# antarcticrainforest/seabreeze_param

Hardware: AMD Instinct MI355X
Metric: grid-points/sec for sea_breeze_diag on N2560x1920 global grid; achieved HBM GB/s (higher is better)
Workload: dtype f64; 1 GPU; seabreeze_diag generic flavour, N1280 (2560x1920) global grid, nz=56, fp64 (BASELINE.json configs[2]); stream=torch's current stream (torch and the library share one HIP runtime), plan_cache=stored, nx=2560, ny=1920, nz=56, search_halo=16, parallelism=latband1, variant=default, comm=none, multi_rank_rccl=unmeasured on hardware so far (one GPU per box in the build pool)

## Files before the change

seabreeze_param_amd/csrc/sb_capi.hip:

```cpp
#include "../../include/seabreeze_hip.h"
#include "sb_launch.hpp"

#include <dlfcn.h>
#include <rccl/rccl.h>

#include <algorithm>
#include <chrono>
#include <cmath>
#include <condition_variable>
#include <functional>
#include <mutex>
#include <thread>
#include <cstdio>
#include <cstdlib>
#include <cstring>
#include <string>
#include <vector>

namespace {

thread_local std::string g_err;

struct DevBuf {
    void *p = nullptr;
// ... 198 lines not shown
           c->stats_ngathered == (c->gathered ? c->ngathered : 0);
}

template <typename T>
int run_diag(sb_ctx *c, DiagJob<T> &job, hipStream_t st, int phases = 3) {
    const Geo &g = job.g;
    const size_t ncell = (size_t)g.nxh * g.nyh;
    const size_t nbits = (size_t)g.nyh * g.nw * sizeof(uint64_t);
    int rc;
    if ((rc = ensure(c, c->bandbits, nbits))) return rc;
    if ((rc = ensure(c, c->clsbits, nbits))) return rc;
    const int H = pick_halo(c);
    int txw, tyrows, tx, ty;
    const bool strip32 = H > 16 && sizeof(T) == 4 && !c->no_wide_strip && sb_strip32_shape(g.nx, g.rows, &tx, &ty);
    const bool strip = strip32 || (H <= 16 && sb_strip_shape(g.nx, g.rows, &tx, &ty));
    const int vb = strip32 ? 2 : 1;
    if (strip) { txw = 32; tyrows = 16; }
    else {
        sb_thc_tile_shape(H > 16 ? H : 24, &txw, &tyrows);
        tx = (g.nx + txw - 1) / txw; ty = (g.rows + tyrows - 1) / tyrows;
    }
    const int Hk = strip32 ? 32 : strip ? 16 : (H > 16 ? H : 24);
    const int ntile = strip ? tx * (ty + 2 * vb) : tx * ty;
    const int nflag = ntile + 2;
    if (c->tiles.cap < (size_t)2 * nflag * sizeof(int) || c->tiles_n != nflag || c->tiles_strip != (strip ? vb : 0)) {
        if ((rc = ensure(c, c->tiles, (size_t)2 * nflag * sizeof(int)))) return rc;
        HIPCHK(c, hipMemsetAsync(c->tiles.p, 0, (size_t)2 * nflag * sizeof(int), st));
        c->tiles_n = nflag;
        c->tiles_strip = strip ? vb : 0;
        c->flag_parity = 0;
    }
    int *flags_now = (int *)c->tiles.p + (size_t)c->flag_parity * nflag;
    int *flags_next = (int *)c->tiles.p + (size_t)(1 - c->flag_parity) * nflag;
    job.thc_ty = tyrows; job.thc_ntx = tx; job.thc_nty = ty;
    job.thc_txs = txw == 32 ? 5 : 6;
    job.strip = strip32 ? 2 : strip ? 1 : 0;
    if (strip) { job.tile_sx = ty + 2 * vb; job.tile_sy = 1; job.tile_off = vb; }
    else { job.tile_sx = 1; job.tile_sy = tx; job.tile_off = 0; }
    job.bandbits = (uint64_t *)c->bandbits.p;
    job.clsbits = (uint64_t *)c->clsbits.p;
    job.stats = (const T *)c->stats;
    job.tile_nnmax = flags_now;
    job.counters = flags_now + (size_t)ntile;
    job.ticket = (int *)c->ticket;
// ... 16 lines not shown
        if ((rc = ensure(c, c->nws, (size_t)g.nx * g.ny * sizeof(T)))) return rc;
        if ((rc = ensure(c, c->nwd, (size_t)g.nx * g.ny * sizeof(T)))) return rc;
        job.nws = (T *)c->nws.p;
        job.nwd = (T *)c->nwd.p;
    }
    job.t0 = nullptr;
    if (!job.t0_fly) {
        if ((rc = ensure(c, c->t0, ncell * sizeof(T)))) return rc;
        job.t0 = (T *)c->t0.p;
    }
    if ((rc = ensure(c, c->jobcopy, sizeof(DiagJob<double>)))) return rc;
    job.self = (DiagJob<T> *)c->jobcopy.p;
    job.plan = nullptr; job.plan_gen = nullptr; job.call_id = 0; job.plan_use = 0; job.seg_trust = 0;
    job.moments_out = nullptr; job.stats_ticket = nullptr; job.strip_update = 0;
    if (strip) {
        const size_t need = 64 + (size_t)c->ncu * SB_PLAN_STRIDE;
        if (c->plan.cap < need) {
            if ((rc = ensure(c, c->plan, need))) return rc;
            HIPCHK(c, hipMemsetAsync(c->plan.p, 0, need, st));
            c->plan_bits = nullptr;
        }
        if (phases & 1) {
            if (c->call_seq == 0x7fffffff) {
                HIPCHK(c, hipMemsetAsync(c->plan.p, 0, need, st));
                c->call_seq = 0;
                c->plan_bits = nullptr;
            }
            ++c->call_seq;
            const int key[8] = {g.nx, g.ny, g.h, g.bnd, g.rows, c->ncu, tx, ty | (vb << 24)};
            c->plan_use = c->plan_bits == c->bandbits.p && std::memcmp(key, c->plan_key, sizeof(key)) == 0 ? 1 : 0;
            std::memcpy(c->plan_key, key, sizeof(key));
            c->plan_bits = c->bandbits.p;
        }
        job.plan = (char *)c->plan.p + 64;
        job.plan_gen = (int *)c->plan.p;
        job.call_id = c->call_seq;
        job.plan_use = c->no_plan_cache ? 0 : c->plan_use;
    } else if (phases & 1) c->plan_bits = nullptr;
    job.stamps = nullptr;
#ifdef SB_STAMPS
    if ((rc = ensure(c, c->stamps, (size_t)4096 * SB_NSTAMP * sizeof(long long)))) return rc;
    job.stamps = (long long *)c->stamps.p;
#endif
    SbLaunchCtx lc;
// ... 1356 lines not shown
```

seabreeze_param_amd/csrc/sb_launch.hpp:

```cpp
#pragma once
#include "sb_device.hpp"

#define SB_STATS_MAX_BLOCKS 2048
#define SB_MAX_LDS_HALO 32
#define SB_DIST_TY 4
enum { SB_PROF_SCAN = 0, SB_PROF_WIND = 1, SB_PROF_T0 = 2, SB_PROF_THC = 3, SB_PROF_PREP = 4, SB_PROF_KERNELS = 5 };
#define SB_PROF_EVENTS (2 * SB_PROF_KERNELS)
#ifndef SB_WIND_UN
#define SB_WIND_UN 8
#endif
#ifndef SB_WIND_WGS_PER_CU
#define SB_WIND_WGS_PER_CU 4
#endif
#ifndef SB_WIND_UN_F32
#define SB_WIND_UN_F32 14
#endif
#ifndef SB_WIND_WGS_PER_CU_F32
#define SB_WIND_WGS_PER_CU_F32 8
#endif

struct SbLaunchCtx {
    hipStream_t stream;
    hipEvent_t *prof;
    unsigned *prof_mask;
// ... 14 lines not shown

template <typename T>
hipError_t sb_launch_stats(const T *ary, int nx, int ny, int ld, size_t off0, Moments *partials, T *stats,
                           Moments *moments_out, int *ticket, hipStream_t st);
template <typename T>
hipError_t sb_launch_sigmoid_apply(const T *ary, T *sm, size_t n, const T *stats, hipStream_t st);
template <typename T>
hipError_t sb_launch_diag(const DiagJob<T> &job, int H, const SbLaunchCtx &lc);
void sb_thc_tile_shape(int H, int *tx, int *ty);
template <typename T>
hipError_t sb_launch_thc(const DiagJob<T> &job, int H, int ncu, hipStream_t st);

template <typename T>
hipError_t sb_launch_strip(const DiagJob<T> &job, int ncu, hipStream_t st);
bool sb_strip_shape(int nx, int rows, int *ntx, int *nty);
template <typename T>
hipError_t sb_launch_strip32(const DiagJob<T> &job, int ncu, hipStream_t st);
template <>
hipError_t sb_launch_strip32<float>(const DiagJob<float> &job, int ncu, hipStream_t st);
template <>
hipError_t sb_launch_strip32<double>(const DiagJob<double> &job, int ncu, hipStream_t st);
bool sb_strip32_shape(int nx, int rows, int *ntx, int *nty);

template <typename T>
hipError_t sb_launch_theta_to_t0(T *theta, const T *z, const T *sigma, size_t n, const T *stats, hipStream_t st);

template <typename T>
hipError_t sb_launch_edges(const T *lsm, const T *ci, T *coast, int nx, int ny, int rule, int bnd, hipStream_t st);
template <typename T>
hipError_t sb_launch_dist(const T *coast, const T *mask, const T *phi, const T *lamf,
// ... 15 lines not shown
```

seabreeze_param_amd/csrc/sb_strip_kernel.hip:

```cpp
#include "sb_thc_common.hpp"
#include "sb_strip_common.hpp"

#define STRIP_H 16
#define STRIP_W 64
#define STRIP_SW (STRIP_W - 2 * STRIP_H)
#define STRIP_C 16
#define STRIP_NT 1024
#define STRIP_RING 128
#define STRIP_P (STRIP_W + 1)
#define STRIP_MAXW 768
#define STRIP_SCHED 384
#define STRIP_ROUND 90
#define STRIP_FB 40
#define STRIP_DEPTH 3


#if defined(SB_STAMPS) && !defined(SB_STAMPS_WIND)
#define SB_T(i) do { if (lane == 0) job.stamps[(size_t)(blockIdx.x * (STRIP_NT / SB_WAVE) + wv) * SB_NSTAMP + (i)] = wall_clock64(); } while (0)
#else
#define SB_T(i) do { } while (0)
#endif

__constant__ double sb_strip_k[20] = {
    1.4426950408889634, 0.6931471805599453, 2.3190468138462996e-17, -708.0, 700.0,
    1.6666666666666666e-01, 4.1666666666666664e-02, 8.333333333333333e-03, 1.388888888888889e-03,
    1.984126984126984e-04, 2.48015873015873e-05, 2.7557319223985893e-06, 2.755731922398589e-07,
    2.505210838544172e-08,
// ... 37 lines not shown

#define SB_FIX_BIAS 0x4338000000000000ull
__device__ __forceinline__ u64 sb_to_fixed(double x, sb_cdp k) {
    return (u64)__double_as_longlong(__builtin_fma(x, SB_K(16, 0x1p40), SB_K(17, 0x1.8p52)));
}

template <typename T, bool FLY>
struct StripRegs {
    T th;
    T zz, sg;
    uint32_t lw;
    uint32_t lbit;
};

template <typename T, bool FLY>
__global__ __launch_bounds__(STRIP_NT) void k_strip(char *plan, const int *plan_gen, const Moments *fold_partials, int G, StripJob<T> job) {
    constexpr int H = STRIP_H, W = STRIP_W, SW = STRIP_SW, C = STRIP_C, P = STRIP_P, NWV = STRIP_NT / SB_WAVE;
    constexpr int RM = STRIP_RING - 1;
    static_assert(NWV == C && SW == 32, "one staged row per wave, 32 owned columns");
    static_assert(STRIP_SCHED == SB_PLAN_SCHED, "a stored plan holds one round's steps");
    __shared__ u64 sA[STRIP_RING * P];
    __shared__ u64 sL[STRIP_RING * P];
    __shared__ unsigned short sC[STRIP_RING * P];
    __shared__ u64 s_land[STRIP_RING];
    __shared__ u64 s_bits[STRIP_MAXW];
    __shared__ uint2 s_ent[STRIP_SCHED];
    __shared__ unsigned short s_cell[3][SW * C];
    __shared__ Moments s_wpart[NWV];
    __shared__ int s_scan[NWV];
    __shared__ int s_misc[12];
    __shared__ T s_sdr[2];
    static_assert(sizeof(u64) * (2 * STRIP_RING * P + STRIP_RING + STRIP_MAXW) + 2 * STRIP_RING * P + 8 * STRIP_SCHED +
                          6 * SW * C + sizeof(Moments) * NWV + 4 * NWV + 48 + 16 <= 160 * 1024,
                  "k_strip: LDS of one workgroup");

    const Geo g = job.g;
    const int tid = threadIdx.x, lane = tid & 63;
    const int wv = __builtin_amdgcn_readfirstlane(tid >> 6);
    const int npad = job.nty + 2;
    const int npos = job.ntx * npad;
    const unsigned npad_magic = 0xffffffffu / (unsigned)npad + 1u;

    SB_T(0);
    T sd = T(0), rr = T(0);
    Moments pm = moments_empty();
    double shift_c = 0.0;
    const bool fold_stats = job.fold && job.fold_nparts > 0;
    if (fold_stats) {
        if (tid < job.fold_nparts) pm = fold_partials[tid];
        shift_c = (double)job.sigma[(size_t)g.h * g.nxh + g.h];
    } else if (FLY && job.ngath > 0) {
        if (wv == 0) {
            Moments m = moments_empty();
            for (int b = lane; b < job.ngath; b += SB_WAVE) m = moments_merge(m, job.gath[b]);
// ... 4 lines not shown
                s_sdr[0] = st4[0]; s_sdr[1] = st4[1];
                if (blockIdx.x == 0) { for (int i = 0; i < 4; ++i) job.stats_out[i] = st4[i]; }
            }
        }
    } else if (FLY) { sd = job.stats[0]; rr = job.stats[1]; }
    const int nch = (npos + STRIP_NT - 1) / STRIP_NT;
    const int nwords = nch * NWV;
    typedef const __attribute__((address_space(4))) int *cintp;
    char *const plan_wg = plan + (size_t)blockIdx.x * SB_PLAN_STRIDE;
    unsigned *const plan_lists = (unsigned *)(plan_wg + SB_PLAN_LIST_OFF);
    const uint2 plan_ent = ((const uint2 *)(plan_wg + SB_PLAN_ENT_OFF))[tid < STRIP_SCHED ? tid : 0];
    const int plan_stored = ((cintp)plan_wg)[0], plan_nst = min(((cintp)plan_wg)[1], STRIP_SCHED);
    const int plan_rb = ((cintp)plan_wg)[2], plan_re = ((cintp)plan_wg)[3];
    const bool cached = job.plan_use != 0 && plan_stored != 0 && *(cintp)plan_gen <= plan_stored;
    auto load_plane = [&]() {
        u64 mine = 0;
        for (int base = 0; base < nch; base += 8) {
            int f[8];
#pragma unroll
            for (int j = 0; j < 8; ++j) {
                const int i = (base + j) * STRIP_NT + tid;
                f[j] = job.flags[i < npos ? i : npos - 1];
            }
#pragma unroll
            for (int j = 0; j < 8; ++j) {
                const int i = (base + j) * STRIP_NT + tid;
                mine |= (i < npos && f[j] != 0) ? 1ull << (base + j) : 0ull;
            }
        }
        for (int c = 0; c < nch; ++c) {
            const u64 b = __builtin_amdgcn_ballot_w64((mine >> c) & 1ull);
            if (lane == 0) s_bits[c * NWV + wv] = b;
        }
    };
    if (__builtin_expect(!cached, 0)) load_plane();
    else {
        if (tid < plan_nst) s_ent[tid] = plan_ent;
        if (tid == 0) { s_misc[0] = plan_nst; s_misc[5] = plan_rb; s_misc[6] = plan_re; s_misc[8] = 0; }
    }
    for (int i = tid; i < STRIP_RING; i += STRIP_NT) { sA[i * P] = 0; sL[i * P] = 0; sC[i * P] = 0; }
    if (tid == 0) s_misc[4] = 0;
    if (fold_stats) wave_total_shifted_store(pm, s_wpart);
    SB_T(1);
    __syncthreads();
    SB_T(2);
    unsigned *s_pre = (unsigned *)&s_cell[0][0];
    unsigned *s_cost = (unsigned *)&sA[0];
    constexpr int CW_STAGED = 4, CW_ACTIVE = 2, CW_RUN = 2;
    static_assert(sizeof(s_cell) >= sizeof(unsigned) * STRIP_MAXW, "the prefix array fits where the cell lists lie");
    auto wave_sync = [] { asm volatile("s_waitcnt lgkmcnt(0)" ::: "memory"); };
    auto stage_word = [&](int k) -> u64 {
        const u64 a = s_bits[k], pv = k > 0 ? s_bits[k - 1] : 0ull, nx = k + 1 < nwords ? s_bits[k + 1] : 0ull;
        return a | (a << 1) | (pv >> 63) | (a >> 1) | (nx << 63);
    };
    auto run_starts = [&](int k, u64 sw) -> u64 {
        const u64 swp = k > 0 ? stage_word(k - 1) : 0ull;
        return sw & ~((sw << 1) | (swp >> 63));
    };
    int tot_packed = 0, tot_cost = 0;
    auto make_prefix = [&](bool with_cost) {
        int run = 0, crun = 0;
        for (int k0 = 0; k0 < nwords; k0 += SB_WAVE) {
            const int k = k0 + lane;
            const u64 a = k < nwords ? s_bits[k] : 0ull, sw = k < nwords ? stage_word(k) : 0ull;
            const int v = (int)((unsigned)__popcll(a) | (unsigned)__popcll(sw) << 16);
            const int incl = sb_wave_scan_add(v);
            if (k < nwords) s_pre[k] = (unsigned)(run + incl - v);
            run += __builtin_amdgcn_readlane(incl, SB_WAVE - 1);
// ... 43 lines not shown
                const u64 upto = lane == 63 ? ~0ull : (1ull << (lane + 1)) - 1ull;
                const int cum = __builtin_amdgcn_readlane(lo, src) + CW_STAGED * __popcll(sw & upto) + CW_ACTIVE * __popcll(a & upto) + CW_RUN * __popcll(rs & upto);
                const u64 over = __builtin_amdgcn_ballot_w64(cum > t);
                const int bpos = over ? __ffsll((unsigned long long)over) - 1 : 63;
                return (int)(__builtin_amdgcn_readfirstlane((int)s_pre[kk]) & 0xffff) + __popcll(a & ((1ull << bpos) - 1ull));
            }
        }
        return nact;
    };
    auto make_schedule = [&](int ra, int rb) {
        int n0, n1;
        const int k0w = find_word(ra, false, n0), k1w = find_word(rb - 1, false, n1);
        const int p0 = k0w < 0 ? -1 : k0w * 64 + nth_bit(sb_uniform64(s_bits[k0w < 0 ? 0 : k0w]), n0);
        const int p1 = k1w < 0 ? -1 : k1w * 64 + nth_bit(sb_uniform64(s_bits[k1w < 0 ? 0 : k1w]), n1);
        wave_sync();
        if (p0 < 1 || p1 < p0) { if (lane == 0) s_misc[0] = 0; return; }
        if (lane < STRIP_DEPTH) s_ent[lane] = make_uint2(SCH_DRAIN | SCH_IDLE, 0u);
        if (lane < 3) s_misc[1 + lane] = 0;
        int n_out = STRIP_DEPTH;
        for (int c = p0 - 1; c <= p1 + 1; c += SB_WAVE) {
            const int pp = c + lane;
            unsigned win = 0;
#pragma unroll
            for (int d = 0; d < 5; ++d) {
                const int q = pp + d - 2;
                const bool in = q >= p0 && q <= p1;
                const u64 w = s_bits[in ? q >> 6 : 0];
                win |= (in && ((w >> (q & 63)) & 1ull)) ? 1u << d : 0u;
            }
            const bool st = pp <= p1 + 1 && (win & 0xeu) != 0u;
            const int sp = (int)__umulhi((unsigned)(pp < 0 ? 0 : pp), npad_magic), jpp = pp - sp * npad;
            const bool st_prev = (win & 0x7u) != 0u && jpp != 0, st_next = (win & 0x1cu) != 0u && jpp != npad - 1;
            const bool en = st && !st_next;
            const u64 ms = __builtin_amdgcn_ballot_w64(st), me = __builtin_amdgcn_ballot_w64(en);
            const u64 below = (1ull << lane) - 1ull;
            const int at = n_out + __popcll(ms & below) + __popcll(me & below);
            n_out += __popcll(ms) + __popcll(me);
            if (st) {
                const unsigned sjv = ((unsigned)sp << 16) | (unsigned)jpp;
                const unsigned e = (unsigned)pp | ((win & 1u) ? SCH_Q2 : 0u) | (st_prev ? 0u : SCH_RESTART);
                if (at < STRIP_SCHED) s_ent[at] = make_uint2(e, sjv);
                if (en && at + 1 < STRIP_SCHED) s_ent[at + 1] = make_uint2((unsigned)pp | SCH_DRAIN | ((win & 2u) ? SCH_Q1 : 0u), sjv);
            }
        }
        n_out = min(n_out, STRIP_SCHED - 2);
        const int n_pad = (n_out + STRIP_DEPTH - 1) / STRIP_DEPTH * STRIP_DEPTH;
        wave_sync();
        const unsigned last_sj = s_ent[n_out - 1].y;
        if (lane < n_pad - n_out) s_ent[n_out + lane] = make_uint2(SCH_DRAIN | SCH_IDLE, last_sj);
        if (lane == 0) s_misc[0] = n_pad;
    };
    if (__builtin_expect(!cached, 0)) {
        if (wv == 0) {
            make_prefix(true);
            const int rb0 = act_before_cost((int)(((long long)blockIdx.x * tot_cost) / G));
            const int re0 = blockIdx.x + 1 == (unsigned)G ? (tot_packed & 0xffff) : act_before_cost((int)(((long long)(blockIdx.x + 1) * tot_cost) / G));
            if (lane == 0) { s_misc[5] = rb0; s_misc[6] = re0; s_misc[0] = 0; }
// ... 9 lines not shown
                const u64 m = __builtin_amdgcn_ballot_w64(q);
                const int qi = nq + __popcll(m & ((1ull << lane) - 1ull));
                nq += __popcll(m);
                if (q) v.x |= (unsigned)(qi & (SB_PLAN_NQ - 1)) << SCH_QI_SHIFT;
                if (i < nstv) { s_ent[i] = v; eg[i] = v; }
            }
            const bool ok = re0 - rb0 <= STRIP_ROUND && nq <= SB_PLAN_NQ;
            if (lane == 0) {
                int *h = (int *)plan_wg;
                h[1] = nstv; h[2] = rb0; h[3] = re0;
                h[0] = ok ? job.call_id : 0;
                s_misc[8] = ok ? 1 : 0;
            }
        }
        __syncthreads();
        if (tid < 8) sA[tid * P] = 0;
        SB_T(3);
    }
    const bool store_lists = __builtin_amdgcn_readfirstlane(s_misc[8]) != 0;
    unsigned qc = ~0u;
    const unsigned qc_off = (unsigned)(min(wv, C / 2 - 1) * SB_WAVE + lane);
    const int r_begin = __builtin_amdgcn_readfirstlane(s_misc[5]), r_end = __builtin_amdgcn_readfirstlane(s_misc[6]);

    const bool fastx = g.nx > W + 2;
    const bool limited = g.bnd == BND_HALO;
    const int big_reach = 1 << 20;
    auto frame_reach = [&](int x, int y) __attribute__((always_inline)) -> int {
        const int rx = (g.band & GEO_BAND_EW) ? big_reach : min(x + g.h, g.nx - 1 - x + g.h);
        const int rs = (g.band & GEO_BAND_SOUTH) ? big_reach : y + g.h, rn = (g.band & GEO_BAND_NORTH) ? big_reach : g.ny - 1 - y + g.h;
        return min(rx, min(rs, rn));
    };
// ... 16 lines not shown
            else if (fastx) {
                if (g.bnd == BND_WRAPPER) {
                    int m = xs + 1;
                    m = m < 0 ? m + g.nx : (m >= g.nx ? m - g.nx : m);
                    Xc = (m < 1 ? 1 : m) - 1;
                } else Xc = xs < 0 ? xs + g.nx : (xs >= g.nx ? xs - g.nx : xs);
            } else {
                int Yd;
                sb_map_cell(g, xs, 0, Xc, Yd);
            }
            const unsigned xc = ok ? (unsigned)Xc : 0u;
            cc_colb = xc * (unsigned)sizeof(T);
            cc_clsb = (xc >> 5) * 4u;
            cc_lbit = ok ? 1u << (xc & 31u) : 0u;
        }
        const int ys = (jp - 1) * C + wv;
        int Yr;
        bool rowok = true;
        if (g.bnd == BND_HALO) {
            int yw = ys;
            if ((g.band & GEO_BAND_SOUTH) && yw < 0) yw = 0;
            if ((g.band & GEO_BAND_NORTH) && yw >= g.ny) yw = g.ny - 1;
            Yr = yw + g.h; rowok = Yr >= 0 && Yr < g.nyh; Yr = rowok ? Yr : 0;
        }
        else Yr = ys < 0 ? 0 : (ys >= g.ny ? g.ny - 1 : ys);
        const size_t rowb = (size_t)((unsigned)Yr * (unsigned)g.nxh) * sizeof(T), wordb = (size_t)((unsigned)Yr * (unsigned)g.nw) * 8u;
        R.th = *(const T *)((const char *)job.theta + rowb + cc_colb);
        if constexpr (FLY) {
            R.zz = *(const T *)((const char *)job.z + rowb + cc_colb);
            R.sg = *(const T *)((const char *)job.sigma + rowb + cc_colb);
        }
// ... 54 lines not shown
        } else if (!cached) {
            unsigned short *tab = sC + o;
            unsigned v[C];
#pragma unroll
            for (int i = 0; i < C; ++i) v[i] = tab[i * P];
            unsigned cc = (unsigned)carry;
#pragma unroll
            for (int i = 0; i < C; ++i) { cc += v[i]; tab[i * P] = (unsigned short)cc; }
            carry = cc;
        }
    };

    struct BandWords { u64 a0, b0, a1, b1, c0, c1; int sh; };
    auto band_issue = [&](int strip, int jp) __attribute__((always_inline)) -> BandWords {
        const int k = max(wv - C / 2, 0);
        const int y0 = (jp - 1) * C + 2 * k;
        const int ya = min(max(y0, 0), g.ny - 1), yb = min(max(y0 + 1, 0), g.ny - 1);
        const int xa = strip * SW + g.h;
        const int wlo = xa >> 6, whi = min(wlo + 1, g.nw - 1);
        cu64p bits = (cu64p)job.bandbits;
        BandWords w;
        w.a0 = bits[(size_t)(ya + g.h) * g.nw + wlo]; w.b0 = bits[(size_t)(ya + g.h) * g.nw + whi];
        w.a1 = bits[(size_t)(yb + g.h) * g.nw + wlo]; w.b1 = bits[(size_t)(yb + g.h) * g.nw + whi];
        w.sh = xa & 63;
        w.c0 = w.c1 = 0;
        if (g.bnd == BND_WRAPPER && strip == job.ntx - 1) {
            cu64p cls = (cu64p)job.clsbits;
            const int wl = (g.nx - 1 + g.h) >> 6;
            w.c0 = cls[(size_t)(ya + g.h) * g.nw + wl]; w.c1 = cls[(size_t)(yb + g.h) * g.nw + wl];
        }
        return w;
    };

    const unsigned cell_code = (unsigned)((2 * max(wv - C / 2, 0) + (lane >> 5)) << 5 | (lane & (SW - 1)));
    auto list_cells = [&](int strip, int jp, const BandWords &bwd, int buf) __attribute__((always_inline)) {
        const int y0 = (jp - 1) * C + 2 * max(wv - C / 2, 0);
        const int ncol = min(g.nx - strip * SW, SW);
        const unsigned colmask = ncol >= 32 ? 0xffffffffu : (1u << ncol) - 1u;
        auto row_bits = [&](u64 a, u64 b2, int y) -> unsigned {
            const u64 f = bwd.sh ? (a >> bwd.sh) | (b2 << (64 - bwd.sh)) : a;
            return (y >= 0 && y < g.rows) ? (unsigned)f & colmask : 0u;
        };
        const u64 m = (u64)row_bits(bwd.a0, bwd.b0, y0) | (u64)row_bits(bwd.a1, bwd.b1, y0 + 1) << 32;
        if (m == 0) return;
        unsigned code = cell_code;
        if (g.bnd == BND_WRAPPER && strip == job.ntx - 1) {
            if (strip * SW + (int)(lane & (SW - 1)) == g.nx - 1) {
                const unsigned sl = (unsigned)((g.nx - 1 + g.h) & 63);
                code |= 1u << 10 | (unsigned)(((lane >> 5) ? (bwd.c1 >> sl) : (bwd.c0 >> sl)) & 1ull) << 9;
            }
        }
// ... 16 lines not shown
            nl = (int)((code >> 15) & 2047u);
            own = ((code >> 9) & 1u) != 0u;
            found = valid && nn != 0;
            nn = max(nn, 1);
        }
        if (__builtin_expect(!cached, 0)) {
            const int ncell = __builtin_amdgcn_readfirstlane(s_misc[1 + buf]);
            const int e = wv * SB_WAVE + lane;
            valid = e < ncell;
            code = s_cell[buf][valid ? e : 0];
            if (wv * SB_WAVE >= ncell) {
                if (store_lists) plan_lists[qi * (unsigned)(SW * C) + (unsigned)e] = ~0u;
                return;
            }
        }
        const int lx = (int)(code & 31u), ly = (int)((code >> 5) & 15u);
        const int x = strip * SW + lx, y = (jp - 1) * C + ly;
        const unsigned o = (unsigned)y * (unsigned)g.nx + (unsigned)x;
        const unsigned rho = (unsigned)(jp * C + ly);
        const unsigned cx = (unsigned)(lx + H + 1);
        if (__builtin_expect(!cached, 0)) {
            int lim = H;
            if (limited) lim = min(lim, frame_reach(x, y));
            const int limc = max(lim, 1);
            auto count = [&](int rad) __attribute__((always_inline)) {
                const unsigned r1 = __umul24((rho + rad) & RM, P) + cx, r0 = __umul24((rho - rad - 1) & RM, P) + cx;
                return (int)(unsigned short)((unsigned)sC[r1 + rad] - (unsigned)sC[r0 + rad] - (unsigned)sC[r1 - rad - 1] + (unsigned)sC[r0 - rad - 1]);
            };
            int nl1[4];
#pragma unroll
            for (int k = 0; k < 4; ++k) nl1[k] = count(limited ? min(4 * (k + 1), limc) : 4 * (k + 1));
            int lo = 1, hi = limc;
// ... 43 lines not shown

    auto finish_stats = [&]() {
        if (wv == 0) {
            const Moments m = moments_of_shifted(shift_c, block_total_shifted_finish<NWV>(s_wpart));
            T st4[4];
            sigmoid_scalars<T>(m, st4);
            if (lane == 0) {
                s_sdr[0] = st4[0]; s_sdr[1] = st4[1];
                if (blockIdx.x == 0) { for (int i = 0; i < 4; ++i) job.stats_out[i] = st4[i]; }
            }
        }
    };
    if (fold_stats && r_begin >= r_end && blockIdx.x == 0) finish_stats();
    for (int ra = r_begin; ra < r_end; ra += STRIP_ROUND) {
        if (ra > r_begin) {
            if (wv == 0) { make_prefix(false); make_schedule(ra, min(ra + STRIP_ROUND, r_end)); }
            __syncthreads();
        }
        const int nst = __builtin_amdgcn_readfirstlane(s_misc[0]);
        if (nst == 0) break;
        auto entry = [&](int i, unsigned &e, unsigned &j) __attribute__((always_inline)) {
            const uint2 v = s_ent[i < nst ? i : nst - 1];
            e = i < nst ? (unsigned)__builtin_amdgcn_readfirstlane((int)v.x) : (SCH_DRAIN | SCH_IDLE);
            j = (unsigned)__builtin_amdgcn_readfirstlane((int)v.y);
        };
        unsigned E0, J0, E1, J1, E2, J2;
        SB_T(28);
        entry(STRIP_DEPTH, E0, J0); entry(STRIP_DEPTH + 1, E1, J1); entry(STRIP_DEPTH + 2, E2, J2);
        StripRegs<T, FLY> R0, R1, R2;
        SB_T(29);
        issue(R0, J0);
        SB_T(30);
        issue(R1, J1); issue(R2, J2);
        SB_T(31);
        if (fold_stats && ra == r_begin) finish_stats();
        SB_T(4);
        auto step = [&](StripRegs<T, FLY> &R, unsigned &E, unsigned &J, const unsigned &En, int i, int buf) __attribute__((always_inline)) {
            const unsigned ent = E, sj = J;
#if defined(SB_STAMPS) && !defined(SB_STAMPS_WIND)
            if (i < SB_NSTAMP - 5) SB_T(5 + i);
#endif
            entry(i + STRIP_DEPTH, E, J);
            const int pos = (int)(ent & 0xffffu);
            const int strip = (int)(sj >> 16), jp = (int)(sj & 0xffffu);
            const bool drain = (ent & SCH_DRAIN) != 0, idle = (ent & SCH_IDLE) != 0;
            const int qoff = drain ? 1 : 2;
            const bool qany = (ent & (drain ? SCH_Q1 : SCH_Q2)) != 0;
            if (!idle) {
                if (ent & SCH_RESTART) {
                    lds_barrier();
                    if (FLY && (fold_stats || job.ngath > 0)) { sd = s_sdr[0]; rr = s_sdr[1]; }
                }
                BandWords bwd;
                const bool lister = qany && wv >= C / 2 && !cached;
                if (lister) bwd = band_issue(strip, jp - qoff);
                if (tid == STRIP_NT - 1) s_misc[1 + (buf == 2 ? 0 : buf + 1)] = 0;
                if (!drain) stage(R, ent, jp);
                if (lister) list_cells(strip, jp - qoff, bwd, buf);
            }
            unsigned qn = ~0u;
            if (cached) qn = plan_lists[((En >> SCH_QI_SHIFT) & (SB_PLAN_NQ - 1)) * (unsigned)(SW * C) + qc_off];
            issue(R, J);
            if (!idle) {
                lds_barrier();
                if (qany && wv < C / 2) query(pos - qoff, strip, jp - qoff, buf, (ent >> SCH_QI_SHIFT) & (SB_PLAN_NQ - 1));
                if (!drain && wv >= 5 && wv < 8) vertical(jp);
            }
            if (cached) qc = qn;
        };
        for (int i = STRIP_DEPTH; i < nst; i += STRIP_DEPTH) {
            step(R0, E0, J0, E1, i, 0);
            step(R1, E1, J1, E2, i + 1, 1);
            step(R2, E2, J2, E0, i + 2, 2);
        }
        __syncthreads();
    }

    SB_T(5);
    auto slow_cell = [&](const DiagJob<T> &cj, int x, int y, int &nnmax) __attribute__((always_inline)) {
        const unsigned o = (unsigned)y * (unsigned)g.nx + (unsigned)x;
// ... 6 lines not shown
        const T mulg = sb_bit(cj.clsbits, g.nw, x + g.h, y + g.h) ? T(1) : T(-1);
        job.thc[o] = mulg * cg;
    };
    if (s_misc[4] != 0 && cached) {
        const DiagJob<T> &cj = *job.cold;
        int *s_qblk = (int *)&s_cell[0][0];
        __syncthreads();
        if (tid == 0) s_misc[9] = 0;
        __syncthreads();
        const int nstp = s_misc[0];
        for (int i = tid; i < nstp; i += STRIP_NT) {
            const uint2 v = s_ent[i];
            const bool dr = (v.x & SCH_DRAIN) != 0u;
            if (!(v.x & SCH_IDLE) && (v.x & (dr ? SCH_Q1 : SCH_Q2)) != 0u) {
                const int qi = (int)((v.x >> SCH_QI_SHIFT) & (SB_PLAN_NQ - 1));
                s_qblk[qi] = (int)((v.y & 0xffff0000u) | ((v.y & 0xffffu) - (dr ? 1u : 2u)));
                atomicMax(&s_misc[9], qi + 1);
            }
        }
        __syncthreads();
        const int nq = s_misc[9];
        for (int q = 0; q < nq; ++q) {
            const unsigned code = tid < SW * C ? plan_lists[(unsigned)q * (unsigned)(SW * C) + (unsigned)tid] : ~0u;
            if (code != ~0u && ((code >> 10) & 31u) == 0u) {
                const int blk = s_qblk[q];
                const int strip = blk >> 16, jp = blk & 0xffff;
                int nnmax = 0;
                slow_cell(cj, strip * SW + (int)(code & 31u), (jp - 1) * C + (int)((code >> 5) & 15u), nnmax);
                if (nnmax > 1) atomicMax(&job.flags[strip * npad + jp], nnmax);
            }
        }
        __syncthreads();
    } else if (s_misc[4] != 0) {
        const DiagJob<T> &cj = *job.cold;
        if (wv == 0) make_prefix(false);
        __syncthreads();
        tot_packed = s_misc[7];
        for (int r = r_begin; r < r_end; ++r) {
            int n;
            const int kw = find_word(r, false, n);
            if (kw < 0) break;
            const int pos = kw * 64 + nth_bit(sb_uniform64(s_bits[kw]), n);
            const int strip = pos / npad, jp = pos - strip * npad;
            int nnmax = 0;
            if (tid < SW * C) {
                const int x = strip * SW + (tid & (SW - 1)), y = (jp - 1) * C + (tid >> 5);
                if (x < g.nx && y >= 0 && y < g.rows && sb_bit(job.bandbits, g.nw, x + g.h, y + g.h)) {
                    const unsigned o = (unsigned)y * (unsigned)g.nx + (unsigned)x;
                    if (strip_is_mark(job.thc[o])) slow_cell(cj, x, y, nnmax);
                }
            }
            if (nnmax > 1) atomicMax(&job.flags[pos], nnmax);
        }
    }
    SB_T(6);
    if (job.update) {
        __syncthreads();
        const DiagJob<T> &cj = *job.cold;
        auto apply = [&](unsigned o) __attribute__((always_inline)) {
            const T n_thc = __hip_atomic_load(&job.thc[o], __ATOMIC_RELAXED, __HIP_MEMORY_SCOPE_AGENT);
            sb_trigger_update<T, false>(cj, (size_t)o, n_thc, sb_trigger_load<T>(cj, (size_t)o));
        };
        if (cached || store_lists) {
            int *s_qblk = (int *)&s_cell[0][0];
            if (tid == 0) s_misc[9] = 0;
            __syncthreads();
            const int nstp = s_misc[0];
            for (int i = tid; i < nstp; i += STRIP_NT) {
                const uint2 v = s_ent[i];
                const bool dr = (v.x & SCH_DRAIN) != 0u;
                if (!(v.x & SCH_IDLE) && (v.x & (dr ? SCH_Q1 : SCH_Q2)) != 0u) {
                    const int qi = (int)((v.x >> SCH_QI_SHIFT) & (SB_PLAN_NQ - 1));
                    s_qblk[qi] = (int)((v.y & 0xffff0000u) | ((v.y & 0xffffu) - (dr ? 1u : 2u)));
                    atomicMax(&s_misc[9], qi + 1);
                }
            }
            __syncthreads();
            const int nrows = s_misc[9] * (C / 2);
            for (int r0 = wv; r0 < nrows; r0 += 4 * NWV) {
                unsigned code[4];
#pragma unroll
                for (int k = 0; k < 4; ++k) {
                    const int r = r0 + k * NWV;
                    code[k] = ~0u;
                    if (r < nrows) code[k] = __hip_atomic_load(&plan_lists[(unsigned)(r >> 3) * (unsigned)(SW * C) + (unsigned)((r & 7) * SB_WAVE + lane)],
                                                               __ATOMIC_RELAXED, __HIP_MEMORY_SCOPE_AGENT);
                }
#pragma unroll
                for (int k = 0; k < 4; ++k) {
                    if (code[k] == ~0u) continue;
                    const int blk = s_qblk[(r0 + k * NWV) >> 3];
                    const int x = (blk >> 16) * SW + (int)(code[k] & 31u), y = ((blk & 0xffff) - 1) * C + (int)((code[k] >> 5) & 15u);
                    apply((unsigned)y * (unsigned)g.nx + (unsigned)x);
                }
            }
        } else {
            if (wv == 0) make_prefix(false);
            __syncthreads();
            tot_packed = s_misc[7];
            for (int r = r_begin; r < r_end; ++r) {
                int n;
                const int kw = find_word(r, false, n);
                if (kw < 0) break;
                const int pos = kw * 64 + nth_bit(sb_uniform64(s_bits[kw]), n);
                const int strip = pos / npad, jp = pos - strip * npad;
                if (tid < SW * C) {
                    const int x = strip * SW + (tid & (SW - 1)), y = (jp - 1) * C + (tid >> 5);
                    if (x < g.nx && y >= 0 && y < g.rows && sb_bit(job.bandbits, g.nw, x + g.h, y + g.h))
                        apply((unsigned)y * (unsigned)g.nx + (unsigned)x);
                }
            }
        }
    }
    if (job.fold && !(cached && job.lists_stand)) {
        const unsigned nseg = (unsigned)g.nyh * (unsigned)g.nw;
        const unsigned cap = (unsigned)job.seg_cap;
        for (int part = G - 1 - (int)blockIdx.x; part < SB_SEG_PARTS; part += G) {
            if (part < 0) break;
            const unsigned s0 = (unsigned)part * cap, s1 = min(s0 + cap, nseg);
            const unsigned per = (cap + STRIP_NT - 1) / STRIP_NT;
            const unsigned a0 = min(s0 + (unsigned)tid * per, s1), a1 = min(a0 + per, s1);
            int cnt = 0;
// ... 22 lines not shown
    s.ntx = job.thc_ntx; s.nty = job.thc_nty;
    s.fold = job.fold; s.fold_nparts = job.fold_nparts; s.ngath = job.ngath; s.seg_cap = job.seg_cap;
    s.lists_stand = job.lists_stand;
    s.stats = job.stats; s.stats_out = job.stats_out;
    s.fold_partials = job.fold_partials; s.gath = job.gath;
    s.seg_list = job.seg_list; s.seg_count = job.seg_count;
    s.cold = job.self;
    s.plan = job.plan; s.plan_gen = job.plan_gen; s.call_id = job.call_id; s.plan_use = job.plan_use;
    s.update = job.strip_update;
    s.stamps = job.stamps;
    return s;
}

template <typename T>
hipError_t sb_launch_strip(const DiagJob<T> &job, int ncu, hipStream_t st) {
    const dim3 gr(ncu), bl(STRIP_NT);
    const StripJob<T> sj = strip_job<T>(job);
    if (!job.wind_final) return hipErrorInvalidValue;
    if (job.t0_fly) hipLaunchKernelGGL((k_strip<T, true>), gr, bl, 0, st, sj.plan, sj.plan_gen, sj.fold_partials, ncu, sj);
    else hipLaunchKernelGGL((k_strip<T, false>), gr, bl, 0, st, sj.plan, sj.plan_gen, sj.fold_partials, ncu, sj);
    return hipGetLastError();
}
template hipError_t sb_launch_strip<float>(const DiagJob<float> &, int, hipStream_t);
template hipError_t sb_launch_strip<double>(const DiagJob<double> &, int, hipStream_t);

bool sb_strip_shape(int nx, int rows, int *ntx, int *nty) {
    *ntx = (nx + STRIP_SW - 1) / STRIP_SW;
    *nty = (rows + STRIP_C - 1) / STRIP_C;
    return (long long)*ntx * (*nty + 2) < (long long)STRIP_MAXW * 64;
}
```

Before: 41.04 billion grid-points/s.

## Halve strip block height and workgroup size to run two strip workgroups per CU

Shrinks the strip kernel's blocks from 16 to 8 rows, uses 512 threads per workgroup and a smaller LDS ring, and launches twice as many workgroups as CUs so two can be resident on each compute unit. The halo is now two blocks deep, so the schedule windows, query offsets, padding and tile-flag layout are widened to match. The separate s_bits plane is aliased into the sL table to fit the LDS budget. Because of that aliasing, the plane must be reloaded before each scheduling round and before the slow paths. The intent is more latency hiding and parallelism, at the cost of extra halo work per block and repeated plane loads.

```diff
diff --git a/seabreeze_param_amd/csrc/sb_capi.hip b/seabreeze_param_amd/csrc/sb_capi.hip
--- a/seabreeze_param_amd/csrc/sb_capi.hip
+++ b/seabreeze_param_amd/csrc/sb_capi.hip
@@ -236,8 +236,10 @@
     int txw, tyrows, tx, ty;
     const bool strip32 = H > 16 && sizeof(T) == 4 && !c->no_wide_strip && sb_strip32_shape(g.nx, g.rows, &tx, &ty);
     const bool strip = strip32 || (H <= 16 && sb_strip_shape(g.nx, g.rows, &tx, &ty));
-    const int vb = strip32 ? 2 : 1;
-    if (strip) { txw = 32; tyrows = 16; }
+    const int vb = 2;
+    const int layout = strip32 ? 2 : strip ? 3 : 0;
+    const int nwg = (strip && !strip32) ? sb_strip_workgroups(c->ncu) : c->ncu;
+    if (strip) { txw = 32; tyrows = strip32 ? 16 : sb_strip_block_rows(); }
     else {
         sb_thc_tile_shape(H > 16 ? H : 24, &txw, &tyrows);
         tx = (g.nx + txw - 1) / txw; ty = (g.rows + tyrows - 1) / tyrows;
@@ -245,11 +247,11 @@
     const int Hk = strip32 ? 32 : strip ? 16 : (H > 16 ? H : 24);
     const int ntile = strip ? tx * (ty + 2 * vb) : tx * ty;
     const int nflag = ntile + 2;
-    if (c->tiles.cap < (size_t)2 * nflag * sizeof(int) || c->tiles_n != nflag || c->tiles_strip != (strip ? vb : 0)) {
+    if (c->tiles.cap < (size_t)2 * nflag * sizeof(int) || c->tiles_n != nflag || c->tiles_strip != layout) {
         if ((rc = ensure(c, c->tiles, (size_t)2 * nflag * sizeof(int)))) return rc;
         HIPCHK(c, hipMemsetAsync(c->tiles.p, 0, (size_t)2 * nflag * sizeof(int), st));
         c->tiles_n = nflag;
-        c->tiles_strip = strip ? vb : 0;
+        c->tiles_strip = layout;
         c->flag_parity = 0;
     }
     int *flags_now = (int *)c->tiles.p + (size_t)c->flag_parity * nflag;
@@ -296,7 +298,7 @@
     job.plan = nullptr; job.plan_gen = nullptr; job.call_id = 0; job.plan_use = 0; job.seg_trust = 0;
     job.moments_out = nullptr; job.stats_ticket = nullptr; job.strip_update = 0;
     if (strip) {
-        const size_t need = 64 + (size_t)c->ncu * SB_PLAN_STRIDE;
+        const size_t need = 64 + (size_t)nwg * SB_PLAN_STRIDE;
         if (c->plan.cap < need) {
             if ((rc = ensure(c, c->plan, need))) return rc;
             HIPCHK(c, hipMemsetAsync(c->plan.p, 0, need, st));
@@ -309,7 +311,7 @@
                 c->plan_bits = nullptr;
             }
             ++c->call_seq;
-            const int key[8] = {g.nx, g.ny, g.h, g.bnd, g.rows, c->ncu, tx, ty | (vb << 24)};
+            const int key[8] = {g.nx, g.ny, g.h, g.bnd, g.rows, nwg | (tyrows << 24), tx, ty | (layout << 24)};
             c->plan_use = c->plan_bits == c->bandbits.p && std::memcmp(key, c->plan_key, sizeof(key)) == 0 ? 1 : 0;
             std::memcpy(c->plan_key, key, sizeof(key));
             c->plan_bits = c->bandbits.p;
diff --git a/seabreeze_param_amd/csrc/sb_launch.hpp b/seabreeze_param_amd/csrc/sb_launch.hpp
--- a/seabreeze_param_amd/csrc/sb_launch.hpp
+++ b/seabreeze_param_amd/csrc/sb_launch.hpp
@@ -52,6 +52,8 @@
 template <typename T>
 hipError_t sb_launch_strip(const DiagJob<T> &job, int ncu, hipStream_t st);
 bool sb_strip_shape(int nx, int rows, int *ntx, int *nty);
+int sb_strip_workgroups(int ncu);
+int sb_strip_block_rows();
 template <typename T>
 hipError_t sb_launch_strip32(const DiagJob<T> &job, int ncu, hipStream_t st);
 template <>
diff --git a/seabreeze_param_amd/csrc/sb_strip_kernel.hip b/seabreeze_param_amd/csrc/sb_strip_kernel.hip
--- a/seabreeze_param_amd/csrc/sb_strip_kernel.hip
+++ b/seabreeze_param_amd/csrc/sb_strip_kernel.hip
@@ -4,13 +4,15 @@
 #define STRIP_H 16
 #define STRIP_W 64
 #define STRIP_SW (STRIP_W - 2 * STRIP_H)
-#define STRIP_C 16
-#define STRIP_NT 1024
-#define STRIP_RING 128
+#define STRIP_C 8
+#define STRIP_HB (STRIP_H / STRIP_C)
+#define STRIP_NT 512
+#define STRIP_RING 64
 #define STRIP_P (STRIP_W + 1)
-#define STRIP_MAXW 768
+#define STRIP_MAXW 1536
 #define STRIP_SCHED 384
-#define STRIP_ROUND 90
+#define STRIP_ROUND 60
+#define STRIP_QOFF (STRIP_HB + 1)
 #define STRIP_FB 40
 #define STRIP_DEPTH 3
 
@@ -78,30 +80,32 @@
 };
 
 template <typename T, bool FLY>
-__global__ __launch_bounds__(STRIP_NT) void k_strip(char *plan, const int *plan_gen, const Moments *fold_partials, int G, StripJob<T> job) {
-    constexpr int H = STRIP_H, W = STRIP_W, SW = STRIP_SW, C = STRIP_C, P = STRIP_P, NWV = STRIP_NT / SB_WAVE;
+__global__ __launch_bounds__(STRIP_NT) __attribute__((amdgpu_waves_per_eu(4, 4))) void k_strip(char *plan, const int *plan_gen, const Moments *fold_partials, int G, StripJob<T> job) {
+    constexpr int H = STRIP_H, HB = STRIP_HB, W = STRIP_W, SW = STRIP_SW, C = STRIP_C, P = STRIP_P, NWV = STRIP_NT / SB_WAVE;
+    constexpr int LR = SW * C / SB_WAVE;
     constexpr int RM = STRIP_RING - 1;
-    static_assert(NWV == C && SW == 32, "one staged row per wave, 32 owned columns");
+    static_assert(NWV == C && SW == 32 && HB * C == H && C == 8, "one staged row per wave, 32 owned columns, a halo of whole blocks");
     static_assert(STRIP_SCHED == SB_PLAN_SCHED, "a stored plan holds one round's steps");
     __shared__ u64 sA[STRIP_RING * P];
     __shared__ u64 sL[STRIP_RING * P];
     __shared__ unsigned short sC[STRIP_RING * P];
     __shared__ u64 s_land[STRIP_RING];
-    __shared__ u64 s_bits[STRIP_MAXW];
     __shared__ uint2 s_ent[STRIP_SCHED];
     __shared__ unsigned short s_cell[3][SW * C];
     __shared__ Moments s_wpart[NWV];
     __shared__ int s_scan[NWV];
     __shared__ int s_misc[12];
     __shared__ T s_sdr[2];
-    static_assert(sizeof(u64) * (2 * STRIP_RING * P + STRIP_RING + STRIP_MAXW) + 2 * STRIP_RING * P + 8 * STRIP_SCHED +
-                          6 * SW * C + sizeof(Moments) * NWV + 4 * NWV + 48 + 16 <= 160 * 1024,
-                  "k_strip: LDS of one workgroup");
+    static_assert(sizeof(u64) * (2 * STRIP_RING * P + STRIP_RING) + 2 * STRIP_RING * P + 8 * STRIP_SCHED +
+                          6 * SW * C + sizeof(Moments) * NWV + 4 * NWV + 48 + 16 <= 80 * 1024,
+                  "k_strip: LDS of one workgroup (two live on a compute unit)");
+    u64 *const s_bits = &sL[0];
+    static_assert(sizeof(sL) >= sizeof(u64) * STRIP_MAXW && sizeof(sA) >= 2 * sizeof(unsigned) * STRIP_MAXW, "the plane and the prefix arrays fit in the tables");
 
     const Geo g = job.g;
     const int tid = threadIdx.x, lane = tid & 63;
     const int wv = __builtin_amdgcn_readfirstlane(tid >> 6);
-    const int npad = job.nty + 2;
+    const int npad = job.nty + 2 * HB;
     const int npos = job.ntx * npad;
     const unsigned npad_magic = 0xffffffffu / (unsigned)npad + 1u;
 
@@ -136,7 +140,6 @@
     const int plan_rb = ((cintp)plan_wg)[2], plan_re = ((cintp)plan_wg)[3];
     const bool cached = job.plan_use != 0 && plan_stored != 0 && *(cintp)plan_gen <= plan_stored;
     auto load_plane = [&]() {
-        u64 mine = 0;
         for (int base = 0; base < nch; base += 8) {
             int f[8];
 #pragma unroll
@@ -147,33 +150,30 @@
 #pragma unroll
             for (int j = 0; j < 8; ++j) {
                 const int i = (base + j) * STRIP_NT + tid;
-                mine |= (i < npos && f[j] != 0) ? 1ull << (base + j) : 0ull;
-            }
-        }
-        for (int c = 0; c < nch; ++c) {
-            const u64 b = __builtin_amdgcn_ballot_w64((mine >> c) & 1ull);
-            if (lane == 0) s_bits[c * NWV + wv] = b;
-        }
-    };
+                const u64 b = __builtin_amdgcn_ballot_w64(i < npos && f[j] != 0);
+                if (lane == 0 && base + j < nch) s_bits[(base + j) * NWV + wv] = b;
+            }
+        }
+    };
+    auto zero_columns = [&]() { for (int i = tid; i < STRIP_RING; i += STRIP_NT) { sA[i * P] = 0; sL[i * P] = 0; sC[i * P] = 0; } };
     if (__builtin_expect(!cached, 0)) load_plane();
     else {
         if (tid < plan_nst) s_ent[tid] = plan_ent;
         if (tid == 0) { s_misc[0] = plan_nst; s_misc[5] = plan_rb; s_misc[6] = plan_re; s_misc[8] = 0; }
+        zero_columns();
     }
-    for (int i = tid; i < STRIP_RING; i += STRIP_NT) { sA[i * P] = 0; sL[i * P] = 0; sC[i * P] = 0; }
     if (tid == 0) s_misc[4] = 0;
     if (fold_stats) wave_total_shifted_store(pm, s_wpart);
     SB_T(1);
     __syncthreads();
     SB_T(2);
-    unsigned *s_pre = (unsigned *)&s_cell[0][0];
     unsigned *s_cost = (unsigned *)&sA[0];
+    unsigned *s_pre = s_cost + STRIP_MAXW;
     constexpr int CW_STAGED = 4, CW_ACTIVE = 2, CW_RUN = 2;
-    static_assert(sizeof(s_cell) >= sizeof(unsigned) * STRIP_MAXW, "the prefix array fits where the cell lists lie");
     auto wave_sync = [] { asm volatile("s_waitcnt lgkmcnt(0)" ::: "memory"); };
     auto stage_word = [&](int k) -> u64 {
         const u64 a = s_bits[k], pv = k > 0 ? s_bits[k - 1] : 0ull, nx = k + 1 < nwords ? s_bits[k + 1] : 0ull;
-        return a | (a << 1) | (pv >> 63) | (a >> 1) | (nx << 63);
+        return a | (a << 1) | (pv >> 63) | (a << 2) | (pv >> 62) | (a >> 1) | (nx << 63) | (a >> 2) | (nx << 62);
     };
     auto run_starts = [&](int k, u64 sw) -> u64 {
         const u64 swp = k > 0 ? stage_word(k - 1) : 0ull;
@@ -247,23 +247,23 @@
         const int p0 = k0w < 0 ? -1 : k0w * 64 + nth_bit(sb_uniform64(s_bits[k0w < 0 ? 0 : k0w]), n0);
         const int p1 = k1w < 0 ? -1 : k1w * 64 + nth_bit(sb_uniform64(s_bits[k1w < 0 ? 0 : k1w]), n1);
         wave_sync();
-        if (p0 < 1 || p1 < p0) { if (lane == 0) s_misc[0] = 0; return; }
+        if (p0 < HB || p1 < p0) { if (lane == 0) s_misc[0] = 0; return; }
         if (lane < STRIP_DEPTH) s_ent[lane] = make_uint2(SCH_DRAIN | SCH_IDLE, 0u);
         if (lane < 3) s_misc[1 + lane] = 0;
         int n_out = STRIP_DEPTH;
-        for (int c = p0 - 1; c <= p1 + 1; c += SB_WAVE) {
+        for (int c = p0 - HB; c <= p1 + HB; c += SB_WAVE) {
             const int pp = c + lane;
             unsigned win = 0;
 #pragma unroll
-            for (int d = 0; d < 5; ++d) {
-                const int q = pp + d - 2;
+            for (int d = 0; d < 2 * HB + 3; ++d) {
+                const int q = pp + d - (HB + 1);
                 const bool in = q >= p0 && q <= p1;
                 const u64 w = s_bits[in ? q >> 6 : 0];
                 win |= (in && ((w >> (q & 63)) & 1ull)) ? 1u << d : 0u;
             }
-            const bool st = pp <= p1 + 1 && (win & 0xeu) != 0u;
+            const bool st = pp <= p1 + HB && (win & 0x3eu) != 0u;
             const int sp = (int)__umulhi((unsigned)(pp < 0 ? 0 : pp), npad_magic), jpp = pp - sp * npad;
-            const bool st_prev = (win & 0x7u) != 0u && jpp != 0, st_next = (win & 0x1cu) != 0u && jpp != npad - 1;
+            const bool st_prev = (win & 0x1fu) != 0u && jpp != 0, st_next = (win & 0x7cu) != 0u && jpp != npad - 1;
             const bool en = st && !st_next;
             const u64 ms = __builtin_amdgcn_ballot_w64(st), me = __builtin_amdgcn_ballot_w64(en);
             const u64 below = (1ull << lane) - 1ull;
@@ -271,9 +271,9 @@
             n_out += __popcll(ms) + __popcll(me);
             if (st) {
                 const unsigned sjv = ((unsigned)sp << 16) | (unsigned)jpp;
-                const unsigned e = (unsigned)pp | ((win & 1u) ? SCH_Q2 : 0u) | (st_prev ? 0u : SCH_RESTART);
+                const unsigned e = ((win & 1u) && jpp > HB ? SCH_Q2 : 0u) | (st_prev ? 0u : SCH_RESTART);
                 if (at < STRIP_SCHED) s_ent[at] = make_uint2(e, sjv);
-                if (en && at + 1 < STRIP_SCHED) s_ent[at + 1] = make_uint2((unsigned)pp | SCH_DRAIN | ((win & 2u) ? SCH_Q1 : 0u), sjv);
+                if (en && at + 1 < STRIP_SCHED) s_ent[at + 1] = make_uint2(SCH_DRAIN | ((win & 2u) ? SCH_Q1 : 0u), sjv);
             }
         }
         n_out = min(n_out, STRIP_SCHED - 2);
@@ -313,7 +313,7 @@
             }
         }
         __syncthreads();
-        if (tid < 8) sA[tid * P] = 0;
+        zero_columns();
         SB_T(3);
     }
     const bool store_lists = __builtin_amdgcn_readfirstlane(s_misc[8]) != 0;
@@ -360,7 +360,7 @@
             cc_clsb = (xc >> 5) * 4u;
             cc_lbit = ok ? 1u << (xc & 31u) : 0u;
         }
-        const int ys = (jp - 1) * C + wv;
+        const int ys = (jp - HB) * C + wv;
         int Yr;
         bool rowok = true;
         if (g.bnd == BND_HALO) {
@@ -445,7 +445,7 @@
     struct BandWords { u64 a0, b0, a1, b1, c0, c1; int sh; };
     auto band_issue = [&](int strip, int jp) __attribute__((always_inline)) -> BandWords {
         const int k = max(wv - C / 2, 0);
-        const int y0 = (jp - 1) * C + 2 * k;
+        const int y0 = (jp - HB) * C + 2 * k;
         const int ya = min(max(y0, 0), g.ny - 1), yb = min(max(y0 + 1, 0), g.ny - 1);
         const int xa = strip * SW + g.h;
         const int wlo = xa >> 6, whi = min(wlo + 1, g.nw - 1);
@@ -465,7 +465,7 @@
 
     const unsigned cell_code = (unsigned)((2 * max(wv - C / 2, 0) + (lane >> 5)) << 5 | (lane & (SW - 1)));
     auto list_cells = [&](int strip, int jp, const BandWords &bwd, int buf) __attribute__((always_inline)) {
-        const int y0 = (jp - 1) * C + 2 * max(wv - C / 2, 0);
+        const int y0 = (jp - HB) * C + 2 * max(wv - C / 2, 0);
         const int ncol = min(g.nx - strip * SW, SW);
         const unsigned colmask = ncol >= 32 ? 0xffffffffu : (1u << ncol) - 1u;
         auto row_bits = [&](u64 a, u64 b2, int y) -> unsigned {
@@ -512,8 +512,8 @@
                 return;
             }
         }
-        const int lx = (int)(code & 31u), ly = (int)((code >> 5) & 15u);
-        const int x = strip * SW + lx, y = (jp - 1) * C + ly;
+        const int lx = (int)(code & 31u), ly = (int)((code >> 5) & (unsigned)(C - 1));
+        const int x = strip * SW + lx, y = (jp - HB) * C + ly;
         const unsigned o = (unsigned)y * (unsigned)g.nx + (unsigned)x;
         const unsigned rho = (unsigned)(jp * C + ly);
         const unsigned cx = (unsigned)(lx + H + 1);
@@ -587,7 +587,11 @@
     if (fold_stats && r_begin >= r_end && blockIdx.x == 0) finish_stats();
     for (int ra = r_begin; ra < r_end; ra += STRIP_ROUND) {
         if (ra > r_begin) {
+            load_plane();
+            __syncthreads();
             if (wv == 0) { make_prefix(false); make_schedule(ra, min(ra + STRIP_ROUND, r_end)); }
+            __syncthreads();
+            zero_columns();
             __syncthreads();
         }
         const int nst = __builtin_amdgcn_readfirstlane(s_misc[0]);
@@ -614,10 +618,9 @@
             if (i < SB_NSTAMP - 5) SB_T(5 + i);
 #endif
             entry(i + STRIP_DEPTH, E, J);
-            const int pos = (int)(ent & 0xffffu);
             const int strip = (int)(sj >> 16), jp = (int)(sj & 0xffffu);
             const bool drain = (ent & SCH_DRAIN) != 0, idle = (ent & SCH_IDLE) != 0;
-            const int qoff = drain ? 1 : 2;
+            const int qoff = drain ? HB : STRIP_QOFF;
             const bool qany = (ent & (drain ? SCH_Q1 : SCH_Q2)) != 0;
             if (!idle) {
                 if (ent & SCH_RESTART) {
@@ -636,7 +639,7 @@
             issue(R, J);
             if (!idle) {
                 lds_barrier();
-                if (qany && wv < C / 2) query(pos - qoff, strip, jp - qoff, buf, (ent >> SCH_QI_SHIFT) & (SB_PLAN_NQ - 1));
+                if (qany && wv < C / 2) query(strip * npad + jp - qoff, strip, jp - qoff, buf, (ent >> SCH_QI_SHIFT) & (SB_PLAN_NQ - 1));
                 if (!drain && wv >= 5 && wv < 8) vertical(jp);
             }
             if (cached) qc = qn;
@@ -673,7 +676,7 @@
             const bool dr = (v.x & SCH_DRAIN) != 0u;
             if (!(v.x & SCH_IDLE) && (v.x & (dr ? SCH_Q1 : SCH_Q2)) != 0u) {
                 const int qi = (int)((v.x >> SCH_QI_SHIFT) & (SB_PLAN_NQ - 1));
-                s_qblk[qi] = (int)((v.y & 0xffff0000u) | ((v.y & 0xffffu) - (dr ? 1u : 2u)));
+                s_qblk[qi] = (int)((v.y & 0xffff0000u) | ((v.y & 0xffffu) - (dr ? (unsigned)HB : (unsigned)STRIP_QOFF)));
                 atomicMax(&s_misc[9], qi + 1);
             }
         }
@@ -685,13 +688,16 @@
                 const int blk = s_qblk[q];
                 const int strip = blk >> 16, jp = blk & 0xffff;
                 int nnmax = 0;
-                slow_cell(cj, strip * SW + (int)(code & 31u), (jp - 1) * C + (int)((code >> 5) & 15u), nnmax);
+                slow_cell(cj, strip * SW + (int)(code & 31u), (jp - HB) * C + (int)((code >> 5) & (unsigned)(C - 1)), nnmax);
                 if (nnmax > 1) atomicMax(&job.flags[strip * npad + jp], nnmax);
             }
         }
         __syncthreads();
     } else if (s_misc[4] != 0) {
         const DiagJob<T> &cj = *job.cold;
+        __syncthreads();
+        load_plane();
+        __syncthreads();
         if (wv == 0) make_prefix(false);
         __syncthreads();
         tot_packed = s_misc[7];
@@ -703,7 +709,7 @@
             const int strip = pos / npad, jp = pos - strip * npad;
             int nnmax = 0;
             if (tid < SW * C) {
-                const int x = strip * SW + (tid & (SW - 1)), y = (jp - 1) * C + (tid >> 5);
+                const int x = strip * SW + (tid & (SW - 1)), y = (jp - HB) * C + (tid >> 5);
                 if (x < g.nx && y >= 0 && y < g.rows && sb_bit(job.bandbits, g.nw, x + g.h, y + g.h)) {
                     const unsigned o = (unsigned)y * (unsigned)g.nx + (unsigned)x;
                     if (strip_is_mark(job.thc[o])) slow_cell(cj, x, y, nnmax);
@@ -730,30 +736,32 @@
                 const bool dr = (v.x & SCH_DRAIN) != 0u;
                 if (!(v.x & SCH_IDLE) && (v.x & (dr ? SCH_Q1 : SCH_Q2)) != 0u) {
                     const int qi = (int)((v.x >> SCH_QI_SHIFT) & (SB_PLAN_NQ - 1));
-                    s_qblk[qi] = (int)((v.y & 0xffff0000u) | ((v.y & 0xffffu) - (dr ? 1u : 2u)));
+                    s_qblk[qi] = (int)((v.y & 0xffff0000u) | ((v.y & 0xffffu) - (dr ? (unsigned)HB : (unsigned)STRIP_QOFF)));
                     atomicMax(&s_misc[9], qi + 1);
                 }
             }
             __syncthreads();
-            const int nrows = s_misc[9] * (C / 2);
+            const int nrows = s_misc[9] * LR;
             for (int r0 = wv; r0 < nrows; r0 += 4 * NWV) {
                 unsigned code[4];
 #pragma unroll
                 for (int k = 0; k < 4; ++k) {
                     const int r = r0 + k * NWV;
                     code[k] = ~0u;
-                    if (r < nrows) code[k] = __hip_atomic_load(&plan_lists[(unsigned)(r >> 3) * (unsigned)(SW * C) + (unsigned)((r & 7) * SB_WAVE + lane)],
+                    if (r < nrows) code[k] = __hip_atomic_load(&plan_lists[(unsigned)(r / LR) * (unsigned)(SW * C) + (unsigned)((r % LR) * SB_WAVE + lane)],
                                                                __ATOMIC_RELAXED, __HIP_MEMORY_SCOPE_AGENT);
                 }
 #pragma unroll
                 for (int k = 0; k < 4; ++k) {
                     if (code[k] == ~0u) continue;
-                    const int blk = s_qblk[(r0 + k * NWV) >> 3];
-                    const int x = (blk >> 16) * SW + (int)(code[k] & 31u), y = ((blk & 0xffff) - 1) * C + (int)((code[k] >> 5) & 15u);
+                    const int blk = s_qblk[(r0 + k * NWV) / LR];
+                    const int x = (blk >> 16) * SW + (int)(code[k] & 31u), y = ((blk & 0xffff) - HB) * C + (int)((code[k] >> 5) & (unsigned)(C - 1));
                     apply((unsigned)y * (unsigned)g.nx + (unsigned)x);
                 }
             }
         } else {
+            load_plane();
+            __syncthreads();
             if (wv == 0) make_prefix(false);
             __syncthreads();
             tot_packed = s_misc[7];
@@ -764,7 +772,7 @@
                 const int pos = kw * 64 + nth_bit(sb_uniform64(s_bits[kw]), n);
                 const int strip = pos / npad, jp = pos - strip * npad;
                 if (tid < SW * C) {
-                    const int x = strip * SW + (tid & (SW - 1)), y = (jp - 1) * C + (tid >> 5);
+                    const int x = strip * SW + (tid & (SW - 1)), y = (jp - HB) * C + (tid >> 5);
                     if (x < g.nx && y >= 0 && y < g.rows && sb_bit(job.bandbits, g.nw, x + g.h, y + g.h))
                         apply((unsigned)y * (unsigned)g.nx + (unsigned)x);
                 }
@@ -817,11 +825,12 @@
 
 template <typename T>
 hipError_t sb_launch_strip(const DiagJob<T> &job, int ncu, hipStream_t st) {
-    const dim3 gr(ncu), bl(STRIP_NT);
+    const int nwg = sb_strip_workgroups(ncu);
+    const dim3 gr(nwg), bl(STRIP_NT);
     const StripJob<T> sj = strip_job<T>(job);
     if (!job.wind_final) return hipErrorInvalidValue;
-    if (job.t0_fly) hipLaunchKernelGGL((k_strip<T, true>), gr, bl, 0, st, sj.plan, sj.plan_gen, sj.fold_partials, ncu, sj);
-    else hipLaunchKernelGGL((k_strip<T, false>), gr, bl, 0, st, sj.plan, sj.plan_gen, sj.fold_partials, ncu, sj);
+    if (job.t0_fly) hipLaunchKernelGGL((k_strip<T, true>), gr, bl, 0, st, sj.plan, sj.plan_gen, sj.fold_partials, nwg, sj);
+    else hipLaunchKernelGGL((k_strip<T, false>), gr, bl, 0, st, sj.plan, sj.plan_gen, sj.fold_partials, nwg, sj);
     return hipGetLastError();
 }
 template hipError_t sb_launch_strip<float>(const DiagJob<float> &, int, hipStream_t);
@@ -830,5 +839,9 @@
 bool sb_strip_shape(int nx, int rows, int *ntx, int *nty) {
     *ntx = (nx + STRIP_SW - 1) / STRIP_SW;
     *nty = (rows + STRIP_C - 1) / STRIP_C;
-    return (long long)*ntx * (*nty + 2) < (long long)STRIP_MAXW * 64;
+    const long long npad = *nty + 2 * STRIP_HB;
+    return (long long)*ntx * npad < (long long)STRIP_MAXW * 64 && npad < 0x8000;
 }
+
+int sb_strip_workgroups(int ncu) { return 2 * ncu; }
+int sb_strip_block_rows() { return STRIP_C; }
```

Result: no change. 40.92 billion grid-points/s (-0.3%).
